# jabberjabberjabber/video-3d-pipeline

Measured on AMD Instinct MI355X. Metric: 1080p_sbs_to_4k_depth_frames_per_s, higher is better.
Workload: dtype int16 (SGM) + f64 (guided filter sums; f32 depth in/out)

## Files before the change

### video-3d-pipeline_amd/csrc/v3d_guided.hip

```cpp
#include "v3d_common.h"
#include <type_traits>

__device__ __forceinline__ double gf_rcp(double x)
{
    double r = __builtin_amdgcn_rcp(x);
    r = fma(r, fma(-x, r, 1.0), r);
    r = fma(r, fma(-x, r, 1.0), r);
    return r;
}

template <typename TD> __device__ __forceinline__ float gf_ld(const TD* p, size_t i);
template <> __device__ __forceinline__ float gf_ld<float>(const float* p, size_t i) { const float v = p[i]; return fabsf(v) <= 3.402823466e38f ? v : 0.f; }
template <> __device__ __forceinline__ float gf_ld<int16_t>(const int16_t* p, size_t i) { const int d = p[i]; return d > 0 ? (float)d * 0.0625f : 0.f; }
template <> __device__ __forceinline__ float gf_ld<uint16_t>(const uint16_t* p, size_t i) { return (float)p[i]; }

typedef unsigned short v3d_u16x2v __attribute__((ext_vector_type(2)));
typedef unsigned short v3d_u16x4 __attribute__((ext_vector_type(4)));
__device__ __forceinline__ void gf_st(float* p, float q) { *p = q; }
__device__ __forceinline__ void gf_st(uint16_t* p, float q) { *p = v3d_rint_u16(q); }

#define GF_TX 64
#define GF_RUN 8
#define GF_RMAX 16

template <typename TD>
__device__ __forceinline__ double gf_bilinear(const TD* __restrict__ src, int Ws, int Hs, double sx, double sy, int x, int y)
{
    const double fx = (x + 0.5) * sx - 0.5, fy = (y + 0.5) * sy - 0.5;
    const double x0f = floor(fx), y0f = floor(fy);
    const double wx = fx - x0f, wy = fy - y0f;
    const int x0 = (int)x0f, y0 = (int)y0f;
    const int xa = min(max(x0, 0), Ws - 1), xb = min(max(x0 + 1, 0), Ws - 1);
    const int ya = min(max(y0, 0), Hs - 1), yb = min(max(y0 + 1, 0), Hs - 1);
    const double top = (double)gf_ld(src, (size_t)ya * Ws + xa) * (1.0 - wx) + (double)gf_ld(src, (size_t)ya * Ws + xb) * wx;
    const double bot = (double)gf_ld(src, (size_t)yb * Ws + xa) * (1.0 - wx) + (double)gf_ld(src, (size_t)yb * Ws + xb) * wx;
    return top * (1.0 - wy) + bot * wy;
}

template <int SWEEP, int GF_RUNY, typename TD, typename TO>
__global__ __launch_bounds__(256) void k_gf(const TD* __restrict__ depth_lo, int Wlo, int Hlo,
                                            const uint8_t* __restrict__ guide, int W, int H, int r, double eps,
                                            double* __restrict__ A, double* __restrict__ B, TO* __restrict__ out)
{
    constexpr int NS = SWEEP == 1 ? 4 : 2;
    constexpr int GF_TY = 4 * GF_RUNY;
    extern __shared__ __attribute__((aligned(16))) double smem[];
    const int rows = GF_TY + 2 * r;
    const int pitch = (GF_TX + 2 * r) | 1;
    const int hp = GF_TX + 1;
    double* t0 = smem;
    double* t1 = t0 + rows * pitch;
    double* hs = t1 + rows * pitch;

    const int tid = threadIdx.x;
    const int ox = blockIdx.x * GF_TX, oy = blockIdx.y * GF_TY;
    const double sx = (double)Wlo / (double)W, sy = (double)Hlo / (double)H;

    const int tw = GF_TX + 2 * r;
    for (int i = tid; i < rows * tw; i += 256) {
        const int ty = i / tw, tx = i - ty * tw;
        const int gx = ox - r + tx, gy = oy - r + ty;
        double v0 = 0.0, v1 = 0.0;
        if (gx >= 0 && gx < W && gy >= 0 && gy < H) {
            if (SWEEP == 1) {
                v0 = (double)guide[(size_t)gy * W + gx] / 255.0;
                v1 = gf_bilinear(depth_lo, Wlo, Hlo, sx, sy, gx, gy);
            } else {
                v0 = A[(size_t)gy * W + gx];
                v1 = B[(size_t)gy * W + gx];
            }
        }
        t0[ty * pitch + tx] = v0;
        t1[ty * pitch + tx] = v1;
    }
    __syncthreads();

    const int nruns = GF_TX / GF_RUN;
    for (int task = tid; task < rows * nruns; task += 256) {
        const int row = task % rows, run = task / rows;
        const double* r0 = t0 + row * pitch + run * GF_RUN;
        const double* r1 = t1 + row * pitch + run * GF_RUN;
        double s0 = 0.0, s1 = 0.0, s2 = 0.0, s3 = 0.0;
        for (int k = 0; k <= 2 * r; k++) {
            const double u = r0[k], v = r1[k];
            s0 += u; s1 += v;
            if (SWEEP == 1) { s2 += u * u; s3 += u * v; }
        }
        double* h = hs + row * hp + run * GF_RUN;
        const int hplane = rows * hp;
        for (int j = 0; j < GF_RUN; j++) {
            h[j] = s0; h[hplane + j] = s1;
            if (SWEEP == 1) { h[2 * hplane + j] = s2; h[3 * hplane + j] = s3; }
            if (j + 1 < GF_RUN) {
                const double un = r0[j + 2 * r + 1], vn = r1[j + 2 * r + 1];
                const double uo = r0[j], vo = r1[j];
                s0 += un - uo; s1 += vn - vo;
                if (SWEEP == 1) { s2 += un * un - uo * uo; s3 += un * vn - uo * vo; }
            }
        }
    }
    __syncthreads();

    {
        const int x = tid % GF_TX, runy = tid / GF_TX;
        const int hplane = rows * hp;
        const double* h = hs + (runy * GF_RUNY) * hp + x;
        double s[NS];
#pragma unroll
        for (int q = 0; q < NS; q++) s[q] = 0.0;
        for (int k = 0; k <= 2 * r; k++)
#pragma unroll
            for (int q = 0; q < NS; q++) s[q] += h[q * hplane + k * hp];
        const int gx = ox + x;
        const int cx = min(gx + r, W - 1) - max(gx - r, 0) + 1;
        for (int j = 0; j < GF_RUNY; j++) {
            const int gy = oy + runy * GF_RUNY + j;
            if (gx < W && gy < H) {
                const int cy = min(gy + r, H - 1) - max(gy - r, 0) + 1;
                const double cnt = (double)(cx * cy);
                if (SWEEP == 1) {
                    const double mI = s[0] / cnt, mp = s[1] / cnt, mII = s[2] / cnt, mIp = s[3] / cnt;
                    const double var = mII - mI * mI, cov = mIp - mI * mp;
                    const double a = cov / (var + eps);
                    A[(size_t)gy * W + gx] = a;
                    B[(size_t)gy * W + gx] = mp - a * mI;
                } else {
                    const double I = (double)guide[(size_t)gy * W + gx] / 255.0;
                    const float q = (float)((s[0] / cnt) * I + (s[1] / cnt));
                    if constexpr (std::is_same<TO, float>::value) out[(size_t)gy * W + gx] = q;
                    else out[(size_t)gy * W + gx] = v3d_rint_u16(q);
                }
            }
            if (j + 1 < GF_RUNY) {
                const int kn = j + 2 * r + 1;
#pragma unroll
                for (int q = 0; q < NS; q++) s[q] += h[q * hplane + kn * hp] - h[q * hplane + j * hp];
            }
        }
    }
}

#ifndef GF_CH
#define GF_CH 3
#endif
typedef double v3d_f64x2 __attribute__((ext_vector_type(2)));
typedef float v3d_f32x2 __attribute__((ext_vector_type(2)));
typedef float v3d_f32x4 __attribute__((ext_vector_type(4)));

template <int SWEEP, int RR, typename TD, typename TO>
__global__ __launch_bounds__(256) void k_gfm(const TD* __restrict__ depth_lo, int Wlo, int Hlo,
                                             const uint8_t* __restrict__ guide, int W, int H, double eps, int band_h,
                                             double* __restrict__ A, double* __restrict__ B, TO* __restrict__ out,
                                             size_t depth_stride, size_t guide_stride)
{
    static_assert(RR % 2 == 0, "pairs must not straddle the strip's halo boundary");
    constexpr int R = 2 * RR + 1, NOUT = 256 - 2 * RR;
    __shared__ __attribute__((aligned(16))) double sVd[2][2][2][256];
    __shared__ __attribute__((aligned(16))) int2 sVi[2][2][256];
    {
        const size_t f = blockIdx.z, n4 = (size_t)W * H;
        depth_lo += f * depth_stride; guide += f * guide_stride; A += f * 2 * n4; B += f * 2 * n4; out += f * n4;
    }
    const int tid = threadIdx.x;
    const int gx = blockIdx.x * NOUT - RR + tid;
    const int ya = blockIdx.y * band_h, yb = min(ya + band_h, H);
    const bool col_ok = gx >= 0 && gx < W;
    const double sx = (double)Wlo / (double)W, sy = (double)Hlo / (double)H;
    const int nsteps = (yb - ya) + 2 * RR;

    const int hrow = tid >> 7, hq = tid & 127;
    const int hgx = blockIdx.x * NOUT - RR + 2 * hq;
    const bool pair_in = 2 * hq >= RR && 2 * hq < 256 - RR;
    const bool px0 = pair_in && hgx < W, px1 = pair_in && hgx + 1 < W;
    const bool vec_ok = px1 && (W & 1) == 0;

    int bxa = 0, bxb = 0; double bwx = 0.0;
    if (SWEEP == 1) {
        const double fx = (gx + 0.5) * sx - 0.5, x0f = floor(fx);
        bwx = fx - x0f;
        bxa = min(max((int)x0f, 0), Wlo - 1); bxb = min(max((int)x0f + 1, 0), Wlo - 1);
    }
    double r0[R], r1[R], v0 = 0.0, v1 = 0.0;
    int rg[R], vg = 0, vgg = 0;
#pragma unroll
    for (int j = 0; j < R; j++) { r0[j] = 0.0; r1[j] = 0.0; rg[j] = 0; }

    struct RowIn { int g; float a0, a1, b0, b1; double n0, n1; bool in; };
    const int gxc = min(max(gx, 0), W - 1);
    auto fetch_row = [&](int t) -> RowIn {
        RowIn q; q.g = 0; q.a0 = q.a1 = q.b0 = q.b1 = 0.f; q.n0 = q.n1 = 0.0;
        const int e = ya - RR + t;
        q.in = col_ok && e >= 0 && e < H && t < nsteps;
        const size_t o = (size_t)min(max(e, 0), H - 1) * W + gxc;
        if (SWEEP == 1) {
            q.g = guide[o];
            const double fy = (e + 0.5) * sy - 0.5, y0f = floor(fy);
            const TD* ra = depth_lo + (size_t)min(max((int)y0f, 0), Hlo - 1) * Wlo;
            const TD* rb = depth_lo + (size_t)min(max((int)y0f + 1, 0), Hlo - 1) * Wlo;
            q.a0 = gf_ld(ra, bxa); q.a1 = gf_ld(ra, bxb); q.b0 = gf_ld(rb, bxa); q.b1 = gf_ld(rb, bxb);
        } else {
            q.n0 = __builtin_nontemporal_load(A + o); q.n1 = __builtin_nontemporal_load(B + o);
        }
        return q;
    };
    RowIn nx[2] = { fetch_row(0), fetch_row(1) };

    int buf = 0;
    for (int t0 = 0; t0 < nsteps; t0 += 2 * R) {
#pragma unroll
        for (int s = 0; s < R; s++) {
            const int tA = t0 + 2 * s;
            if (tA < nsteps) {
                const int y0 = ya - 2 * RR + tA;
                const bool emit = y0 >= ya;
                const RowIn cur[2] = { nx[0], nx[1] };
                nx[0] = fetch_row(tA + 2); nx[1] = fetch_row(tA + 3);
#pragma unroll
                for (int rr = 0; rr < 2; rr++) {
                    const int j = (2 * s + rr) % R;
                    if (SWEEP == 1) {
                        int gn = 0; double pn = 0.0;
                        if (cur[rr].in) {
                            gn = cur[rr].g;
                            const int e = ya - RR + tA + rr;
                            const double fy = (e + 0.5) * sy - 0.5, wy = fy - floor(fy);
                            const double a0 = (double)cur[rr].a0, b0 = (double)cur[rr].b0;
                            const double top = fma(bwx, (double)cur[rr].a1 - a0, a0);
                            const double bot = fma(bwx, (double)cur[rr].b1 - b0, b0);
                            pn = fma(wy, bot - top, top);
                        }
                        const int go = rg[j]; const double po = r1[j];
                        rg[j] = gn; r1[j] = pn;
                        vg += gn - go; vgg += gn * gn - go * go;
                        v0 += pn - po; v1 = fma((double)gn, pn, fma(-(double)go, po, v1));
                    } else {
                        const double n0 = cur[rr].in ? cur[rr].n0 : 0.0, n1 = cur[rr].in ? cur[rr].n1 : 0.0;
                        const double o0 = r0[j], o1 = r1[j];
                        r0[j] = n0; r1[j] = n1;
                        v0 += n0 - o0; v1 += n1 - o1;
                    }
                    if (emit) {
                        sVd[buf][rr][0][tid] = v0; sVd[buf][rr][1][tid] = v1;
                        if (SWEEP == 1) sVi[buf][rr][tid] = make_int2(vg, vgg);
                    }
                }
                if (emit) {
                    __syncthreads();
                    const int y = y0 + hrow;
                    if (px0 && y < yb) {
                        double fq[2], lq[2], cq[2];
#pragma unroll
                        for (int q = 0; q < 2; q++) {
                            const v3d_f64x2* d = reinterpret_cast<const v3d_f64x2*>(&sVd[buf][hrow][q][0]) + (hq - RR / 2);
                            double f = 0.0, l = 0.0, c = 0.0;
#pragma unroll
                            for (int ch = 0; ch <= RR; ch += GF_CH) {
                                v3d_f64x2 w[GF_CH];
#pragma unroll
                                for (int i = 0; i < GF_CH; i++) if (ch + i <= RR) w[i] = d[ch + i];
#pragma unroll
                                for (int i = 0; i < GF_CH; i++) if (ch + i <= RR) {
                                    if (ch + i == 0) { f = w[i].x; c = w[i].y; }
                                    else if (ch + i == RR) { c += w[i].x; l = w[i].y; }
                                    else { c += w[i].x; c += w[i].y; }
                                }
                                asm volatile("" : "+v"(c) :: "memory");
                            }
                            fq[q] = f; lq[q] = l; cq[q] = c;
                        }
                        int g0 = 0, gg0 = 0, gl = 0, ggl = 0, cg = 0, cgg = 0;
                        if (SWEEP == 1) {
                            const int4* gi = reinterpret_cast<const int4*>(&sVi[buf][hrow][0]) + (hq - RR / 2);
#pragma unroll
                            for (int ch = 0; ch <= RR; ch += 3) {
                                int4 u[3];
#pragma unroll
                                for (int i = 0; i < 3; i++) if (ch + i <= RR) u[i] = gi[ch + i];
#pragma unroll
                                for (int i = 0; i < 3; i++) if (ch + i <= RR) {
                                    if (ch + i == 0) { g0 = u[i].x; gg0 = u[i].y; cg = u[i].z; cgg = u[i].w; }
                                    else if (ch + i == RR) { cg += u[i].x; cgg += u[i].y; gl = u[i].z; ggl = u[i].w; }
                                    else { cg += u[i].x + u[i].z; cgg += u[i].y + u[i].w; }
                                }
                                asm volatile("" : "+v"(cg), "+v"(cgg) :: "memory");
                            }
                        }
                        const double s0a = cq[0] + fq[0], s0b = cq[0] + lq[0], s1a = cq[1] + fq[1], s1b = cq[1] + lq[1];
                        const int cy = min(y + RR, H - 1) - max(y - RR, 0) + 1;
                        const int cx0 = min(hgx + RR, W - 1) - max(hgx - RR, 0) + 1, cx1 = min(hgx + 1 + RR, W - 1) - max(hgx + 1 - RR, 0) + 1;
                        const double inva = gf_rcp((double)(cx0 * cy)), invb = cx1 == cx0 ? inva : gf_rcp((double)(cx1 * cy));
                        const size_t o = (size_t)y * W + hgx;
                        if (SWEEP == 1) {
                            const int sga = cg + g0, sgb = cg + gl, sgga = cgg + gg0, sggb = cgg + ggl;
                            double ab[2][2];
#pragma unroll
                            for (int n = 0; n < 2; n++) {
                                const double inv = n ? invb : inva;
                                const double mI = (double)(n ? sgb : sga) * (inv * (1.0 / 255.0)), mp = (n ? s0b : s0a) * inv;
                                const double mII = (double)(n ? sggb : sgga) * (inv * (1.0 / 65025.0)), mIp = (n ? s1b : s1a) * (inv * (1.0 / 255.0));
                                const double var = fma(-mI, mI, mII), cov = fma(-mI, mp, mIp);
                                const double a = cov * gf_rcp(var + eps);
                                ab[n][0] = a; ab[n][1] = fma(-a, mI, mp);
                            }
                            if (vec_ok) {
                                v3d_f64x2 va = { ab[0][0], ab[1][0] }, vb = { ab[0][1], ab[1][1] };
                                __builtin_nontemporal_store(va, reinterpret_cast<v3d_f64x2*>(A + o));
                                __builtin_nontemporal_store(vb, reinterpret_cast<v3d_f64x2*>(B + o));
                            } else {
                                A[o] = ab[0][0]; B[o] = ab[0][1];
                                if (px1) { A[o + 1] = ab[1][0]; B[o + 1] = ab[1][1]; }
                            }
                        } else {
                            const double Ia = (double)guide[o] * (1.0 / 255.0);
                            const double Ib = px1 ? (double)guide[o + 1] * (1.0 / 255.0) : 0.0;
                            const float qa = (float)((s0a * inva) * Ia + (s1a * inva)), qb = (float)((s0b * invb) * Ib + (s1b * invb));
                            if (vec_ok && (std::is_same<TO, float>::value || (reinterpret_cast<uintptr_t>(out + o) & 3) == 0)) {
                                if constexpr (std::is_same<TO, float>::value) {
                                    v3d_f32x2 vq = { qa, qb };
                                    __builtin_nontemporal_store(vq, reinterpret_cast<v3d_f32x2*>(out + o));
                                } else {
                                    v3d_u16x2v vq = { v3d_rint_u16(qa), v3d_rint_u16(qb) };
                                    __builtin_nontemporal_store(vq, reinterpret_cast<v3d_u16x2v*>(out + o));
                                }
                            } else {
                                gf_st(out + o, qa);
                                if (px1) gf_st(out + o + 1, qb);
                            }
                        }
                    }
                    buf ^= 1;
                }
            }
        }
    }
}

__device__ __forceinline__ int gf_swz2(int m) { return m ^ ((m >> 3) & 1) ^ ((m >> 4) & 1); }
__device__ __forceinline__ int gf_swz4(int m) { return m ^ ((m >> 4) & 3); }
__device__ __forceinline__ int gf_c8(int c) { return 2 * gf_swz2(c >> 1) + (c & 1); }

template <int RR>
__device__ __forceinline__ void gf_run4(const double* row, int c0, double s[4])
{
    const v3d_f64x2* d = reinterpret_cast<const v3d_f64x2*>(row);
    const int m0 = (c0 - RR) >> 1;
    double c = 0.0, l0 = 0.0, l1 = 0.0, l2 = 0.0, r1 = 0.0, r2 = 0.0, r3 = 0.0;
#pragma unroll
    for (int k0 = 0; k0 < RR + 2; k0 += GF_CH) {
        v3d_f64x2 w[GF_CH];
#pragma unroll
        for (int i = 0; i < GF_CH; i++) if (k0 + i < RR + 2) w[i] = d[gf_swz2(m0 + k0 + i)];
#pragma unroll
        for (int i = 0; i < GF_CH; i++) {
            const int k = k0 + i;
            if (k == 0) { l0 = w[i].x; l1 = w[i].y; c = w[i].x; c += w[i].y; }
            else if (k == 1) { l2 = w[i].x; c += w[i].x; c += w[i].y; }
            else if (k < RR) { c += w[i].x; c += w[i].y; }
            else if (k == RR) { c += w[i].x; r1 = w[i].y; }
            else if (k == RR + 1) { r2 = w[i].x; r3 = w[i].y; }
        }
        asm volatile("" : "+v"(c) :: "memory");
    }
    s[0] = c; s[1] = (s[0] + r1) - l0; s[2] = (s[1] + r2) - l1; s[3] = (s[2] + r3) - l2;
}

template <int RR>
__device__ __forceinline__ void gf_run4(const int2* row, int c0, int2 s[4])
{
    const int4* d = reinterpret_cast<const int4*>(row);
    const int m0 = (c0 - RR) >> 1;
    int2 c = make_int2(0, 0), l0 = c, l1 = c, l2 = c, r1 = c, r2 = c, r3 = c;
#pragma unroll
    for (int k0 = 0; k0 < RR + 2; k0 += 3) {
        int4 w[3];
#pragma unroll
        for (int i = 0; i < 3; i++) if (k0 + i < RR + 2) w[i] = d[gf_swz2(m0 + k0 + i)];
#pragma unroll
        for (int i = 0; i < 3; i++) {
            const int k = k0 + i;
            const int2 a = make_int2(w[i].x, w[i].y), b = make_int2(w[i].z, w[i].w);
            if (k == 0) { l0 = a; l1 = b; c = make_int2(a.x + b.x, a.y + b.y); }
            else if (k == 1) { l2 = a; c.x += a.x + b.x; c.y += a.y + b.y; }
            else if (k < RR) { c.x += a.x + b.x; c.y += a.y + b.y; }
            else if (k == RR) { c.x += a.x; c.y += a.y; r1 = b; }
            else if (k == RR + 1) { r2 = a; r3 = b; }
        }
        asm volatile("" : "+v"(c.x), "+v"(c.y) :: "memory");
    }
    s[0] = c;
    s[1] = make_int2(s[0].x + r1.x - l0.x, s[0].y + r1.y - l0.y);
    s[2] = make_int2(s[1].x + r2.x - l1.x, s[1].y + r2.y - l1.y);
    s[3] = make_int2(s[2].x + r3.x - l2.x, s[2].y + r3.y - l2.y);
}

template <int RR>
__device__ __forceinline__ void gf_run4(const int4* row, int c0, int4 s[4])
{
    int4 c = make_int4(0, 0, 0, 0), l0 = c, l1 = c, l2 = c, r1 = c, r2 = c, r3 = c;
#pragma unroll
    for (int k0 = 0; k0 < 2 * RR + 4; k0 += 3) {
        int4 u[3];
#pragma unroll
        for (int i = 0; i < 3; i++) if (k0 + i < 2 * RR + 4) u[i] = row[gf_swz4(c0 - RR + k0 + i)];
#pragma unroll
        for (int i = 0; i < 3; i++) {
            const int k = k0 + i;
            if (k < 2 * RR + 1) { c.x += u[i].x; c.y += u[i].y; c.z += u[i].z; c.w += u[i].w; }
            if (k == 0) l0 = u[i];
            else if (k == 1) l1 = u[i];
            else if (k == 2) l2 = u[i];
            else if (k == 2 * RR + 1) r1 = u[i];
            else if (k == 2 * RR + 2) r2 = u[i];
            else if (k == 2 * RR + 3) r3 = u[i];
        }
        asm volatile("" : "+v"(c.x), "+v"(c.y), "+v"(c.z), "+v"(c.w) :: "memory");
    }
    s[0] = c;
    s[1] = make_int4(s[0].x - l0.x + r1.x, s[0].y - l0.y + r1.y, s[0].z - l0.z + r1.z, s[0].w - l0.w + r1.w);
    s[2] = make_int4(s[1].x - l1.x + r2.x, s[1].y - l1.y + r2.y, s[1].z - l1.z + r2.z, s[1].w - l1.w + r2.w);
    s[3] = make_int4(s[2].x - l2.x + r3.x, s[2].y - l2.y + r3.y, s[2].z - l2.z + r3.z, s[2].w - l2.w + r3.w);
}

template <int RR>
__device__ __forceinline__ void gf_solve4(const int sg[4], const int sgg[4], const double sp[4], const double sgp[4], int hgx, int y,
                                          int W, int H, double eps, double a[4], double b[4])
{
    const int cy = min(y + RR, H - 1) - max(y - RR, 0) + 1;
    int cx[4];
#pragma unroll
    for (int n = 0; n < 4; n++) cx[n] = min(hgx + n + RR, W - 1) - max(hgx + n - RR, 0) + 1;
    const double inv0 = gf_rcp((double)(cx[0] * cy));
#pragma unroll
    for (int n = 0; n < 4; n++) {
        const double inv = (n == 0 || cx[n] == cx[0]) ? inv0 : gf_rcp((double)(cx[n] * cy));
        const double mI = (double)sg[n] * (inv * (1.0 / 255.0)), mp = sp[n] * inv;
        const double mII = (double)sgg[n] * (inv * (1.0 / 65025.0)), mIp = sgp[n] * (inv * (1.0 / 255.0));
        const double var = fma(-mI, mI, mII), cov = fma(-mI, mp, mIp);
        const double aa = cov * gf_rcp(var + eps);
        a[n] = aa; b[n] = fma(-aa, mI, mp);
    }
}

template <int RR, int COLS, typename TD, bool I1, typename TO>
__global__ __launch_bounds__(2 * COLS, I1 ? 4 : 2) void k_gff(const TD* __restrict__ depth_lo, int Wlo, int Hlo,
                                                const uint8_t* __restrict__ guide, int W, int H, double eps, int band_h,
                                                TO* __restrict__ out, size_t depth_stride, size_t guide_stride)
{
    static_assert(RR % 4 == 0, "runs of four must not straddle the strip's halo boundaries");
    static_assert(!I1 || std::is_same<TD, int16_t>::value, "the integer stage 1 takes the int16 disparity");
    static_assert(COLS == 256 || (COLS == 512 && I1), "strip width (512 columns: I1 only, the f64 route's rows exceed the LDS)");
    constexpr int R = 2 * RR + 1, NOUT = COLS - 4 * RR, HR = COLS / 4;
    constexpr int S1D = 2 * 4 * 2 * COLS * 8, S1 = I1 ? 2 * 4 * COLS * 16 : S1D + 2 * 4 * COLS * 8;
    __shared__ __attribute__((aligned(16))) unsigned char sS1[S1];
    double (*sV1)[4][2][COLS] = reinterpret_cast<double (*)[4][2][COLS]>(sS1);
    int2 (*sVi)[4][COLS] = reinterpret_cast<int2 (*)[4][COLS]>(sS1 + (I1 ? 0 : S1D));
    int4 (*sVq)[4][COLS] = reinterpret_cast<int4 (*)[4][COLS]>(sS1);
    (void)sV1; (void)sVi; (void)sVq;
    __shared__ __attribute__((aligned(16))) double sAB[3][4][2][COLS];
    {
        const size_t f = blockIdx.z, n4 = (size_t)W * H;
        depth_lo += f * depth_stride; guide += f * guide_stride; out += f * n4;
    }
    const int role = __builtin_amdgcn_readfirstlane((int)(threadIdx.x / COLS));
    const int t = threadIdx.x % COLS;
    const int gx0 = blockIdx.x * NOUT - 2 * RR;
    const int gx = gx0 + t;
    const int ya = blockIdx.y * band_h, yb = min(ya + band_h, H);
    const int nrows = (yb - ya) + 4 * RR;
    const int NS = (nrows + 3) >> 2;
    const int NP = NS + 3;

    if (role == 0) {
        const bool col_ok = gx >= 0 && gx < W;
        const int gxc = min(max(gx, 0), W - 1);
        uint32_t ring[R];
        double r1[I1 ? 1 : R];
        uint32_t rgw[I1 ? 1 : (R + 3) / 4];
        int vg = 0, vgg = 0, vP = 0, vgP = 0;
        double v0 = 0.0, v1 = 0.0;
#pragma unroll
        for (int j = 0; j < R; j++) ring[j] = 0u;
#pragma unroll
        for (int j = 0; j < (I1 ? 1 : R); j++) r1[j] = 0.0;
#pragma unroll
        for (int j = 0; j < (I1 ? 1 : (R + 3) / 4); j++) rgw[j] = 0u;
        (void)ring; (void)r1; (void)rgw;
        int bxa, bxb, wxa = 0, wxb = 0; double bwx = 0.0;
        const double sx = (double)Wlo / (double)W, sy = (double)Hlo / (double)H;
        if constexpr (I1) {
            const int kx = gx >> 1;
            bxa = min(max((gx & 1) ? kx : kx - 1, 0), Wlo - 1); bxb = min(max((gx & 1) ? kx + 1 : kx, 0), Wlo - 1);
            wxa = (gx & 1) ? 3 : 1; wxb = 4 - wxa;
        } else {
            const double fx = (gx + 0.5) * sx - 0.5, x0f = floor(fx);
            bwx = fx - x0f;
            bxa = min(max((int)x0f, 0), Wlo - 1); bxb = min(max((int)x0f + 1, 0), Wlo - 1);
        }
        (void)wxa; (void)wxb; (void)bwx;
        struct RowIn { int g; typename std::conditional<I1, int, float>::type a0, a1, b0, b1; bool in; };
        auto fetch_row = [&](int tt) -> RowIn {
            RowIn q;
            const int e = ya - 2 * RR + tt;
            q.in = col_ok && e >= 0 && e < H && tt < nrows;
            const int ec = min(max(e, 0), H - 1);
            q.g = guide[(size_t)ec * W + gxc];
            if constexpr (I1) {
                const int ky = ec >> 1;
                const TD* ra = depth_lo + (size_t)min(max((ec & 1) ? ky : ky - 1, 0), Hlo - 1) * Wlo;
                const TD* rb = depth_lo + (size_t)min(max((ec & 1) ? ky + 1 : ky, 0), Hlo - 1) * Wlo;
                q.a0 = max((int)ra[bxa], 0); q.a1 = max((int)ra[bxb], 0); q.b0 = max((int)rb[bxa], 0); q.b1 = max((int)rb[bxb], 0);
            } else {
                const double fy = (e + 0.5) * sy - 0.5, y0f = floor(fy);
                const TD* ra = depth_lo + (size_t)min(max((int)y0f, 0), Hlo - 1) * Wlo;
                const TD* rb = depth_lo + (size_t)min(max((int)y0f + 1, 0), Hlo - 1) * Wlo;
                q.a0 = gf_ld(ra, bxa); q.a1 = gf_ld(ra, bxb); q.b0 = gf_ld(rb, bxa); q.b1 = gf_ld(rb, bxb);
            }
            return q;
        };
        RowIn nx[4] = { fetch_row(0), fetch_row(1), fetch_row(2), fetch_row(3) };
        for (int p0 = 0; p0 < NP; p0 += R) {
#pragma clang loop unroll(full)
            for (int sp = 0; sp < R; sp++) {
                const int p = p0 + sp;
                if (p < NP) {
                    int tl = t;
                    asm volatile("" : "+v"(tl));
                    const int hrow = tl / HR, c0 = 4 * (tl % HR), hgx = gx0 + c0;
                    const int j = p - 1;
                    if (j >= RR / 2 && j < NS) {
                        const int y = ya - 3 * RR + 4 * j + hrow;
                        double a[4] = { 0.0, 0.0, 0.0, 0.0 }, b[4] = { 0.0, 0.0, 0.0, 0.0 };
                        if (c0 >= RR && c0 < COLS - RR && y >= 0 && y < H && hgx >= 0 && hgx < W) {
                            int sg[4], sgg[4]; double sp_[4], sgp[4];
                            if constexpr (I1) {
                                int4 s[4];
                                gf_run4<RR>(&sVq[j & 1][hrow][0], c0, s);
#pragma unroll
                                for (int n = 0; n < 4; n++) {
                                    sg[n] = s[n].x; sgg[n] = s[n].y;
                                    sp_[n] = (double)s[n].z * (1.0 / 256.0); sgp[n] = (double)s[n].w * (1.0 / 256.0);
                                }
                            } else {
                                int2 si[4];
                                gf_run4<RR>(&sVi[j & 1][hrow][0], c0, si);
                                gf_run4<RR>(&sV1[j & 1][hrow][0][0], c0, sp_);
                                gf_run4<RR>(&sV1[j & 1][hrow][1][0], c0, sgp);
#pragma unroll
                                for (int n = 0; n < 4; n++) { sg[n] = si[n].x; sgg[n] = si[n].y; }
                            }
                            gf_solve4<RR>(sg, sgg, sp_, sgp, hgx, y, W, H, eps, a, b);
#pragma unroll
                            for (int n = 0; n < 4; n++) if (hgx + n >= W) { a[n] = 0.0; b[n] = 0.0; }
                        }
                        double* ab = &sAB[j % 3][hrow][0][0];
                        const int e0 = 2 * gf_swz2(c0 >> 1), e1 = 2 * gf_swz2((c0 >> 1) + 1);
                        *reinterpret_cast<v3d_f64x2*>(ab + e0) = v3d_f64x2{ a[0], a[1] };
                        *reinterpret_cast<v3d_f64x2*>(ab + e1) = v3d_f64x2{ a[2], a[3] };
                        *reinterpret_cast<v3d_f64x2*>(ab + COLS + e0) = v3d_f64x2{ b[0], b[1] };
                        *reinterpret_cast<v3d_f64x2*>(ab + COLS + e1) = v3d_f64x2{ b[2], b[3] };
                    }
                    if (p < NS) {
                        const int tA = 4 * p;
                        const RowIn cur[4] = { nx[0], nx[1], nx[2], nx[3] };
#pragma unroll
                        for (int k = 0; k < 4; k++) nx[k] = fetch_row(tA + 4 + k);
                        const bool emit = p >= RR / 2;
#pragma unroll
                        for (int rr = 0; rr < 4; rr++) {
                            const int slot = (4 * sp + rr) % R;
                            const int e = ya - 2 * RR + tA + rr;
                            if constexpr (I1) {
                                int gn = 0, Pn = 0;
                                if (cur[rr].in) {
                                    gn = cur[rr].g;
                                    const int wya = (e & 1) ? 3 : 1;
                                    Pn = wya * (wxa * cur[rr].a0 + wxb * cur[rr].a1) + (4 - wya) * (wxa * cur[rr].b0 + wxb * cur[rr].b1);
                                }
                                const int go = (int)(ring[slot] & 0xFFu), Po = (int)(ring[slot] >> 8);
                                ring[slot] = ((uint32_t)Pn << 8) | (uint32_t)gn;
                                vg += gn - go; vgg += gn * gn - go * go;
                                vP += Pn - Po; vgP += gn * Pn - go * Po;
                                if (emit) sVq[p & 1][rr][gf_swz4(t)] = make_int4(vg, vgg, vP, vgP);
                            } else {
                                int gn = 0; double pn = 0.0;
                                if (cur[rr].in) {
                                    gn = cur[rr].g;
                                    const double fy = (e + 0.5) * sy - 0.5, wy = fy - floor(fy);
                                    const double a0 = (double)cur[rr].a0, b0 = (double)cur[rr].b0;
                                    const double top = fma(bwx, (double)cur[rr].a1 - a0, a0);
                                    const double bot = fma(bwx, (double)cur[rr].b1 - b0, b0);
                                    pn = fma(wy, bot - top, top);
                                }
                                const int go = (int)((rgw[slot >> 2] >> (8 * (slot & 3))) & 0xFFu); const double po = r1[slot];
                                rgw[slot >> 2] = (rgw[slot >> 2] & ~(0xFFu << (8 * (slot & 3)))) | ((uint32_t)gn << (8 * (slot & 3)));
                                r1[slot] = pn;
                                vg += gn - go; vgg += gn * gn - go * go;
                                v0 += pn - po; v1 = fma((double)gn, pn, fma(-(double)go, po, v1));
                                if (emit) {
                                    const int ct = gf_c8(t);
                                    sV1[p & 1][rr][0][ct] = v0; sV1[p & 1][rr][1][ct] = v1;
                                    sVi[p & 1][rr][ct] = make_int2(vg, vgg);
                                }
                            }
                        }
                    }
                    __syncthreads();
                }
            }
        }
    } else {
        double r0[R], r1[R], va = 0.0, vb = 0.0;
#pragma unroll
        for (int j = 0; j < R; j++) { r0[j] = 0.0; r1[j] = 0.0; }
        for (int p0 = 0; p0 < NP; p0 += R) {
#pragma clang loop unroll(full)
            for (int sp = 0; sp < R; sp++) {
                const int p = p0 + sp;
                if (p < NP) {
                    int tl = t;
                    asm volatile("" : "+v"(tl));
                    const int hrow = tl / HR, c0 = 4 * (tl % HR), hgx = gx0 + c0;
                    {
                        const int j = p - 3;
                        const int y = ya - 4 * RR + 4 * j + hrow;
                        if (j >= RR && j < NS && c0 >= 2 * RR && c0 < COLS - 2 * RR && hgx < W && y < yb) {
                            double sa[4], sb[4];
                            gf_run4<RR>(&sAB[j % 3][hrow][0][0], c0, sa);
                            gf_run4<RR>(&sAB[j % 3][hrow][1][0], c0, sb);
                            const int cy = min(y + RR, H - 1) - max(y - RR, 0) + 1;
                            int cx[4];
#pragma unroll
                            for (int n = 0; n < 4; n++) cx[n] = min(hgx + n + RR, W - 1) - max(hgx + n - RR, 0) + 1;
                            const double inv0 = gf_rcp((double)(cx[0] * cy));
                            const size_t o = (size_t)y * W + hgx;
                            const bool all_in = hgx + 3 < W;
                            const bool vec_ok = all_in && (W & 3) == 0 && ((reinterpret_cast<uintptr_t>(out + o) | reinterpret_cast<uintptr_t>(guide + o)) & 3) == 0
                                                && (reinterpret_cast<uintptr_t>(out + o) & (4 * sizeof(TO) - 1)) == 0;
                            int g[4];
                            if (vec_ok) {
                                const uint32_t g4 = *reinterpret_cast<const uint32_t*>(guide + o);
#pragma unroll
                                for (int n = 0; n < 4; n++) g[n] = (g4 >> (8 * n)) & 0xFF;
                            } else {
#pragma unroll
                                for (int n = 0; n < 4; n++) g[n] = hgx + n < W ? guide[o + n] : 0;
                            }
                            float q[4];
#pragma unroll
                            for (int n = 0; n < 4; n++) {
                                const double inv = (n == 0 || cx[n] == cx[0]) ? inv0 : gf_rcp((double)(cx[n] * cy));
                                const double I = (double)g[n] * (1.0 / 255.0);
                                q[n] = (float)((sa[n] * inv) * I + (sb[n] * inv));
                            }
                            if (vec_ok) {
                                if constexpr (std::is_same<TO, float>::value) {
                                    const v3d_f32x4 vq = { q[0], q[1], q[2], q[3] };
                                    __builtin_nontemporal_store(vq, reinterpret_cast<v3d_f32x4*>(out + o));
                                } else {
                                    const v3d_u16x4 vq = { v3d_rint_u16(q[0]), v3d_rint_u16(q[1]), v3d_rint_u16(q[2]), v3d_rint_u16(q[3]) };
                                    __builtin_nontemporal_store(vq, reinterpret_cast<v3d_u16x4*>(out + o));
                                }
                            } else {
#pragma unroll
                                for (int n = 0; n < 4; n++) if (hgx + n < W) gf_st(out + o + n, q[n]);
                            }
                        }
                    }
                    {
                        const int j = p - 2;
                        if (j >= RR / 2 && j < NS) {
                            const bool emit = j >= RR;
                            double* col = &sAB[j % 3][0][0][gf_c8(tl)];
#pragma unroll
                            for (int rr = 0; rr < 4; rr++) {
                                const int slot = (4 * sp + rr) % R;
                                const double n0 = col[rr * 2 * COLS], n1 = col[rr * 2 * COLS + COLS];
                                const double o0 = r0[slot], o1 = r1[slot];
                                r0[slot] = n0; r1[slot] = n1;
                                va += n0 - o0; vb += n1 - o1;
                                if (emit) { col[rr * 2 * COLS] = va; col[rr * 2 * COLS + COLS] = vb; }
                            }
                        }
                    }
                    __syncthreads();
                }
            }
        }
    }
}

template <int RR, typename TD, typename TO>
static void launch_gff(const TD* depth_lo, int Wlo, int Hlo, const uint8_t* guide, int W, int H, double eps,
                       TO* out, int n, size_t depth_stride, size_t guide_stride, hipStream_t st)
{
    bool i1 = false;
    if constexpr (std::is_same<TD, int16_t>::value) i1 = g_v3d_opt.gf_int1 && W == 2 * Wlo && H == 2 * Hlo;
    const int cols = g_v3d_opt.gf_cols == 512 && i1 ? 512 : 256;
    int band = g_v3d_opt.gf_band;
    if (band <= 0) {
        int dev = 0, ncu = 256;
        (void)hipGetDevice(&dev);
        (void)hipDeviceGetAttribute(&ncu, hipDeviceAttributeMultiprocessorCount, dev);
        const long slots = (long)ncu * (cols == 256 && i1 ? 2 : 1), strips = v3d_cdiv(W, cols - 4 * RR);
        long best = -1;
        for (int nb = 1; nb <= 64 && nb <= H; nb++) {
            const int b = (v3d_cdiv(H, nb) + 1) & ~1;
            const long wgs = strips * v3d_cdiv(H, b) * n, rounds = (wgs + slots - 1) / slots, cost = rounds * (b + 4 * RR);
            if (best < 0 || cost < best) { best = cost; band = b; }
        }
    }
    const dim3 grid(v3d_cdiv(W, cols - 4 * RR), v3d_cdiv(H, band), n);
    if constexpr (std::is_same<TD, int16_t>::value) {
        if (i1 && cols == 512) {
            hipLaunchKernelGGL((k_gff<RR, 512, TD, true, TO>), grid, dim3(1024), 0, st, depth_lo, Wlo, Hlo, guide, W, H, eps, band, out, depth_stride, guide_stride);
            return;
        }
        if (i1) {
            hipLaunchKernelGGL((k_gff<RR, 256, TD, true, TO>), grid, dim3(512), 0, st, depth_lo, Wlo, Hlo, guide, W, H, eps, band, out, depth_stride, guide_stride);
            return;
        }
    }
    hipLaunchKernelGGL((k_gff<RR, 256, TD, false, TO>), grid, dim3(512), 0, st, depth_lo, Wlo, Hlo, guide, W, H, eps, band, out, depth_stride, guide_stride);
}

template <int RR, typename TD, typename TO>
static void launch_gfm(const TD* depth_lo, int Wlo, int Hlo, const uint8_t* guide, int W, int H, double eps,
                       double* A, double* B, TO* out, int n, size_t depth_stride, size_t guide_stride, hipStream_t st)
{
    const int band1 = g_v3d_opt.gf_band1, band2 = g_v3d_opt.gf_band2;
    const dim3 grid1(v3d_cdiv(W, 256 - 2 * RR), v3d_cdiv(H, band1), n), grid2(v3d_cdiv(W, 256 - 2 * RR), v3d_cdiv(H, band2), n);
    hipLaunchKernelGGL((k_gfm<1, RR, TD, TO>), grid1, dim3(256), 0, st, depth_lo, Wlo, Hlo, guide, W, H, eps, band1, A, B, out, depth_stride, guide_stride);
    hipLaunchKernelGGL((k_gfm<2, RR, TD, TO>), grid2, dim3(256), 0, st, depth_lo, Wlo, Hlo, guide, W, H, eps, band2, A, B, out, depth_stride, guide_stride);
}

extern "C" size_t v3d_guided_upscale_ws_bytes(int W, int H)
{
    if (W < 1 || H < 1) return 0;
    return (size_t)W * H * sizeof(double) * 2;
}

static size_t gf_smem(int r, int ns, int ty)
{
    const int rows = ty + 2 * r;
    const int pitch = (GF_TX + 2 * r) | 1;
    return sizeof(double) * ((size_t)2 * rows * pitch + (size_t)ns * rows * (GF_TX + 1));
}

template <typename TD, typename TO>
static int guided_upscale_batch(const TD* depth_lo, int Wlo, int Hlo, size_t depth_stride, const uint8_t* guide,
                                int W, int H, size_t guide_stride, int n, int r, float eps, TO* out, void* ws, void* stream)
{
    if (n < 1) { v3d_set_error("bad batch"); return V3D_ERR_ARG; }
    if (!depth_lo || !guide || !out || !ws) { v3d_set_error("null pointer"); return V3D_ERR_ARG; }
    if (Wlo < 1 || Hlo < 1 || W < 1 || H < 1) { v3d_set_error("bad geometry"); return V3D_ERR_ARG; }
    if (r < 1 || r > GF_RMAX) { v3d_set_error("radius %d outside [1, %d]", r, GF_RMAX); return V3D_ERR_UNSUPPORTED; }
    if (!(eps >= 0.f)) { v3d_set_error("eps must be >= 0"); return V3D_ERR_ARG; }
    if (((uintptr_t)ws & 15) != 0) { v3d_set_error("workspace must be 16-byte aligned"); return V3D_ERR_ARG; }
    hipStream_t st = (hipStream_t)stream;
    double* A = reinterpret_cast<double*>(ws);
    double* B = A + (size_t)W * H;
    if (!g_v3d_opt.gf_tiled && g_v3d_opt.gf_fused && (r == 4 || r == 8)) {
        if (r == 4) launch_gff<4>(depth_lo, Wlo, Hlo, guide, W, H, (double)eps, out, n, depth_stride, guide_stride, st);
        else launch_gff<8>(depth_lo, Wlo, Hlo, guide, W, H, (double)eps, out, n, depth_stride, guide_stride, st);
        V3D_LAUNCH_CHECK();
        return V3D_OK;
    }
    if (!g_v3d_opt.gf_tiled && (r == 4 || r == 8)) {
        if (r == 4) launch_gfm<4>(depth_lo, Wlo, Hlo, guide, W, H, (double)eps, A, B, out, n, depth_stride, guide_stride, st);
        else launch_gfm<8>(depth_lo, Wlo, Hlo, guide, W, H, (double)eps, A, B, out, n, depth_stride, guide_stride, st);
        V3D_LAUNCH_CHECK();
        return V3D_OK;
    }
    for (int f = 0; f < n; f++) {
    const TD* depth_lo_f = depth_lo + (size_t)f * depth_stride; const uint8_t* guide_f = guide + (size_t)f * guide_stride;
    double* A = reinterpret_cast<double*>(ws) + (size_t)f * 2 * W * H; double* B = A + (size_t)W * H; TO* out_f = out + (size_t)f * W * H;
    const int ty = r <= 8 ? 16 : 8;
    const dim3 grid(v3d_cdiv(W, GF_TX), v3d_cdiv(H, ty));
    const size_t sm1 = gf_smem(r, 4, ty), sm2 = gf_smem(r, 2, ty);
    if (ty == 16) {
        V3D_HIP_CHECK(hipFuncSetAttribute((const void*)k_gf<1, 4, TD, TO>, hipFuncAttributeMaxDynamicSharedMemorySize, (int)sm1));
        V3D_HIP_CHECK(hipFuncSetAttribute((const void*)k_gf<2, 4, TD, TO>, hipFuncAttributeMaxDynamicSharedMemorySize, (int)sm2));
        hipLaunchKernelGGL((k_gf<1, 4, TD, TO>), grid, dim3(256), sm1, st, depth_lo_f, Wlo, Hlo, guide_f, W, H, r, (double)eps, A, B, out_f);
        hipLaunchKernelGGL((k_gf<2, 4, TD, TO>), grid, dim3(256), sm2, st, depth_lo_f, Wlo, Hlo, guide_f, W, H, r, (double)eps, A, B, out_f);
    } else {
        V3D_HIP_CHECK(hipFuncSetAttribute((const void*)k_gf<1, 2, TD, TO>, hipFuncAttributeMaxDynamicSharedMemorySize, (int)sm1));
        V3D_HIP_CHECK(hipFuncSetAttribute((const void*)k_gf<2, 2, TD, TO>, hipFuncAttributeMaxDynamicSharedMemorySize, (int)sm2));
        hipLaunchKernelGGL((k_gf<1, 2, TD, TO>), grid, dim3(256), sm1, st, depth_lo_f, Wlo, Hlo, guide_f, W, H, r, (double)eps, A, B, out_f);
        hipLaunchKernelGGL((k_gf<2, 2, TD, TO>), grid, dim3(256), sm2, st, depth_lo_f, Wlo, Hlo, guide_f, W, H, r, (double)eps, A, B, out_f);
    }
    }
    V3D_LAUNCH_CHECK();
    return V3D_OK;
}

extern "C" int v3d_guided_upscale_batch(const float* depth_lo, int Wlo, int Hlo, size_t depth_stride, const uint8_t* guide,
                                        int W, int H, size_t guide_stride, int n, int r, float eps, float* out, void* ws, void* stream)
{
    return guided_upscale_batch<float, float>(depth_lo, Wlo, Hlo, depth_stride, guide, W, H, guide_stride, n, r, eps, out, ws, stream);
}

extern "C" int v3d_guided_upscale(const float* depth_lo, int Wlo, int Hlo, const uint8_t* guide, int W, int H,
                                  int r, float eps, float* out, void* ws, void* stream)
{
    return guided_upscale_batch<float, float>(depth_lo, Wlo, Hlo, 0, guide, W, H, 0, 1, r, eps, out, ws, stream);
}

extern "C" int v3d_guided_upscale_disp16_batch(const int16_t* disp16, int Wlo, int Hlo, size_t disp_stride, const uint8_t* guide,
                                               int W, int H, size_t guide_stride, int n, int r, float eps, float* out, void* ws, void* stream)
{
    return guided_upscale_batch<int16_t, float>(disp16, Wlo, Hlo, disp_stride, guide, W, H, guide_stride, n, r, eps, out, ws, stream);
}

extern "C" int v3d_guided_upscale_u16_batch(const uint16_t* depth_lo, int Wlo, int Hlo, size_t depth_stride, const uint8_t* guide,
                                            int W, int H, size_t guide_stride, int n, int r, float eps, uint16_t* out, void* ws, void* stream)
{
    return guided_upscale_batch<uint16_t, uint16_t>(depth_lo, Wlo, Hlo, depth_stride, guide, W, H, guide_stride, n, r, eps, out, ws, stream);
}
```

Measured before the change: 2563.

## Add interior fast path and scalar row addressing to the guided filter kernel

Adds a wave-uniform interior fast path that uses a precomputed full-window reciprocal instead of per-pixel clipped box counts and f64 reciprocals, in both the coefficient solve and the output stage. The row fetch is restructured to load four rows per step, with scalar (SGPR) row base pointers and 32-bit byte offsets. In the integer route the 2x upsampled bilinear weights are computed once per step from shared horizontal sums using 24-bit multiply-add inline asm, and hrow is made wave-uniform via readfirstlane. This trims VALU address and f64 work in a compute-heavy kernel, at the cost of more inline asm, register pressure and code size.

```diff
diff --git a/video-3d-pipeline_amd/csrc/v3d_guided.hip b/video-3d-pipeline_amd/csrc/v3d_guided.hip
--- a/video-3d-pipeline_amd/csrc/v3d_guided.hip
+++ b/video-3d-pipeline_amd/csrc/v3d_guided.hip
@@ -9,10 +9,22 @@
     return r;
 }
 
-template <typename TD> __device__ __forceinline__ float gf_ld(const TD* p, size_t i);
-template <> __device__ __forceinline__ float gf_ld<float>(const float* p, size_t i) { const float v = p[i]; return fabsf(v) <= 3.402823466e38f ? v : 0.f; }
-template <> __device__ __forceinline__ float gf_ld<int16_t>(const int16_t* p, size_t i) { const int d = p[i]; return d > 0 ? (float)d * 0.0625f : 0.f; }
-template <> __device__ __forceinline__ float gf_ld<uint16_t>(const uint16_t* p, size_t i) { return (float)p[i]; }
+__device__ __forceinline__ float gf_val(float v) { return fabsf(v) <= 3.402823466e38f ? v : 0.f; }
+__device__ __forceinline__ float gf_val(int16_t v) { const int d = v; return d > 0 ? (float)d * 0.0625f : 0.f; }
+__device__ __forceinline__ float gf_val(uint16_t v) { return (float)v; }
+template <typename TD> __device__ __forceinline__ float gf_ld(const TD* p, size_t i) { return gf_val(p[i]); }
+
+#define GF_GLOBAL __attribute__((address_space(1)))
+template <typename T> __device__ __forceinline__ const GF_GLOBAL T* gf_srow(const T* p)
+{
+    const GF_GLOBAL T* g = (const GF_GLOBAL T*)p;
+    asm("" : "+s"(g));
+    return g;
+}
+template <typename T> __device__ __forceinline__ T gf_at(const GF_GLOBAL T* row, uint32_t byte_off)
+{
+    return *reinterpret_cast<const GF_GLOBAL T*>(reinterpret_cast<const GF_GLOBAL char*>(row) + byte_off);
+}
 
 typedef unsigned short v3d_u16x2v __attribute__((ext_vector_type(2)));
 typedef unsigned short v3d_u16x4 __attribute__((ext_vector_type(4)));
@@ -421,6 +433,31 @@
     s[3] = make_int4(s[2].x - l2.x + r3.x, s[2].y - l2.y + r3.y, s[2].z - l2.z + r3.z, s[2].w - l2.w + r3.w);
 }
 
+__device__ __forceinline__ double gf_uniform(double x)
+{
+    const uint64_t v = (uint64_t)__double_as_longlong(x);
+    const uint32_t lo = __builtin_amdgcn_readfirstlane((uint32_t)v), hi = __builtin_amdgcn_readfirstlane((uint32_t)(v >> 32));
+    return __longlong_as_double((long long)(((uint64_t)hi << 32) | lo));
+}
+
+template <int RR>
+__device__ __forceinline__ double gf_inv_full()
+{
+    int n = (2 * RR + 1) * (2 * RR + 1);
+    asm volatile("" : "+v"(n));
+    return gf_uniform(gf_rcp((double)n));
+}
+
+__device__ __forceinline__ void gf_ab(int sg, int sgg, double sp, double sgp, double inv, double inv255, double inv65025,
+                                      double eps, double& a, double& b)
+{
+    const double mI = (double)sg * inv255, mp = sp * inv;
+    const double mII = (double)sgg * inv65025, mIp = sgp * inv255;
+    const double var = fma(-mI, mI, mII), cov = fma(-mI, mp, mIp);
+    const double aa = cov * gf_rcp(var + eps);
+    a = aa; b = fma(-aa, mI, mp);
+}
+
 template <int RR>
 __device__ __forceinline__ void gf_solve4(const int sg[4], const int sgg[4], const double sp[4], const double sgp[4], int hgx, int y,
                                           int W, int H, double eps, double a[4], double b[4])
@@ -429,16 +466,25 @@
     int cx[4];
 #pragma unroll
     for (int n = 0; n < 4; n++) cx[n] = min(hgx + n + RR, W - 1) - max(hgx + n - RR, 0) + 1;
-    const double inv0 = gf_rcp((double)(cx[0] * cy));
+    const double inv0 = gf_rcp((double)__mul24(cx[0], cy));
 #pragma unroll
     for (int n = 0; n < 4; n++) {
-        const double inv = (n == 0 || cx[n] == cx[0]) ? inv0 : gf_rcp((double)(cx[n] * cy));
-        const double mI = (double)sg[n] * (inv * (1.0 / 255.0)), mp = sp[n] * inv;
-        const double mII = (double)sgg[n] * (inv * (1.0 / 65025.0)), mIp = sgp[n] * (inv * (1.0 / 255.0));
-        const double var = fma(-mI, mI, mII), cov = fma(-mI, mp, mIp);
-        const double aa = cov * gf_rcp(var + eps);
-        a[n] = aa; b[n] = fma(-aa, mI, mp);
-    }
+        const double inv = (n == 0 || cx[n] == cx[0]) ? inv0 : gf_rcp((double)__mul24(cx[n], cy));
+        gf_ab(sg[n], sgg[n], sp[n], sgp[n], inv, inv * (1.0 / 255.0), inv * (1.0 / 65025.0), eps, a[n], b[n]);
+    }
+}
+
+__device__ __forceinline__ int gf_mad24(int a, int b, int c)
+{
+    int d;
+    asm("v_mad_i32_i24 %0, %1, %2, %3" : "=v"(d) : "v"(a), "v"(b), "v"(c));
+    return d;
+}
+__device__ __forceinline__ int gf_mad24x3(int a, int c)
+{
+    int d;
+    asm("v_mad_i32_i24 %0, %1, 3, %2" : "=v"(d) : "v"(a), "v"(c));
+    return d;
 }
 
 template <int RR, int COLS, typename TD, bool I1, typename TO>
@@ -450,6 +496,7 @@
     static_assert(!I1 || std::is_same<TD, int16_t>::value, "the integer stage 1 takes the int16 disparity");
     static_assert(COLS == 256 || (COLS == 512 && I1), "strip width (512 columns: I1 only, the f64 route's rows exceed the LDS)");
     constexpr int R = 2 * RR + 1, NOUT = COLS - 4 * RR, HR = COLS / 4;
+    static_assert(HR % 64 == 0, "the lanes of a wave work on one row in the horizontal phases");
     constexpr int S1D = 2 * 4 * 2 * COLS * 8, S1 = I1 ? 2 * 4 * COLS * 16 : S1D + 2 * 4 * COLS * 8;
     __shared__ __attribute__((aligned(16))) unsigned char sS1[S1];
     double (*sV1)[4][2][COLS] = reinterpret_cast<double (*)[4][2][COLS]>(sS1);
@@ -462,13 +509,15 @@
         depth_lo += f * depth_stride; guide += f * guide_stride; out += f * n4;
     }
     const int role = __builtin_amdgcn_readfirstlane((int)(threadIdx.x / COLS));
-    const int t = threadIdx.x % COLS;
+    int t = threadIdx.x % COLS;
+    asm volatile("" : "+v"(t));
     const int gx0 = blockIdx.x * NOUT - 2 * RR;
     const int gx = gx0 + t;
     const int ya = blockIdx.y * band_h, yb = min(ya + band_h, H);
     const int nrows = (yb - ya) + 4 * RR;
     const int NS = (nrows + 3) >> 2;
     const int NP = NS + 3;
+    const double invF = gf_inv_full<RR>();
 
     if (role == 0) {
         const bool col_ok = gx >= 0 && gx < W;
@@ -485,39 +534,48 @@
 #pragma unroll
         for (int j = 0; j < (I1 ? 1 : (R + 3) / 4); j++) rgw[j] = 0u;
         (void)ring; (void)r1; (void)rgw;
-        int bxa, bxb, wxa = 0, wxb = 0; double bwx = 0.0;
+        uint32_t oxg = (uint32_t)gxc, oxa, oxb; double bwx = 0.0;
         const double sx = (double)Wlo / (double)W, sy = (double)Hlo / (double)H;
         if constexpr (I1) {
             const int kx = gx >> 1;
-            bxa = min(max((gx & 1) ? kx : kx - 1, 0), Wlo - 1); bxb = min(max((gx & 1) ? kx + 1 : kx, 0), Wlo - 1);
-            wxa = (gx & 1) ? 3 : 1; wxb = 4 - wxa;
+            oxa = (uint32_t)min(max((gx & 1) ? kx + 1 : kx - 1, 0), Wlo - 1) * (uint32_t)sizeof(TD);
+            oxb = (uint32_t)min(max(kx, 0), Wlo - 1) * (uint32_t)sizeof(TD);
         } else {
             const double fx = (gx + 0.5) * sx - 0.5, x0f = floor(fx);
             bwx = fx - x0f;
-            bxa = min(max((int)x0f, 0), Wlo - 1); bxb = min(max((int)x0f + 1, 0), Wlo - 1);
-        }
-        (void)wxa; (void)wxb; (void)bwx;
-        struct RowIn { int g; typename std::conditional<I1, int, float>::type a0, a1, b0, b1; bool in; };
-        auto fetch_row = [&](int tt) -> RowIn {
-            RowIn q;
-            const int e = ya - 2 * RR + tt;
-            q.in = col_ok && e >= 0 && e < H && tt < nrows;
-            const int ec = min(max(e, 0), H - 1);
-            q.g = guide[(size_t)ec * W + gxc];
+            oxa = (uint32_t)min(max((int)x0f, 0), Wlo - 1) * (uint32_t)sizeof(TD);
+            oxb = (uint32_t)min(max((int)x0f + 1, 0), Wlo - 1) * (uint32_t)sizeof(TD);
+        }
+        (void)bwx;
+        struct StepIn { int g[4]; typename std::conditional<I1, int, float>::type d[I1 ? 4 : 8][2]; };
+        auto fetch_step = [&](int tt) -> StepIn {
+            StepIn q;
+            const int e0 = ya - 2 * RR + tt;
+            asm volatile("" : "+v"(oxg), "+v"(oxa), "+v"(oxb));
+#pragma unroll
+            for (int k = 0; k < 4; k++) q.g[k] = gf_at(gf_srow(guide + (size_t)min(max(e0 + k, 0), H - 1) * W), oxg);
             if constexpr (I1) {
-                const int ky = ec >> 1;
-                const TD* ra = depth_lo + (size_t)min(max((ec & 1) ? ky : ky - 1, 0), Hlo - 1) * Wlo;
-                const TD* rb = depth_lo + (size_t)min(max((ec & 1) ? ky + 1 : ky, 0), Hlo - 1) * Wlo;
-                q.a0 = max((int)ra[bxa], 0); q.a1 = max((int)ra[bxb], 0); q.b0 = max((int)rb[bxa], 0); q.b1 = max((int)rb[bxb], 0);
+                const int kb = (e0 >> 1) - 1;
+#pragma unroll
+                for (int i = 0; i < 4; i++) {
+                    const auto row = gf_srow(depth_lo + (size_t)min(max(kb + i, 0), Hlo - 1) * Wlo);
+                    q.d[i][0] = max((int)gf_at(row, oxa), 0); q.d[i][1] = max((int)gf_at(row, oxb), 0);
+                }
             } else {
-                const double fy = (e + 0.5) * sy - 0.5, y0f = floor(fy);
-                const TD* ra = depth_lo + (size_t)min(max((int)y0f, 0), Hlo - 1) * Wlo;
-                const TD* rb = depth_lo + (size_t)min(max((int)y0f + 1, 0), Hlo - 1) * Wlo;
-                q.a0 = gf_ld(ra, bxa); q.a1 = gf_ld(ra, bxb); q.b0 = gf_ld(rb, bxa); q.b1 = gf_ld(rb, bxb);
+#pragma unroll
+                for (int k = 0; k < 4; k++) {
+                    const int ec = min(max(e0 + k, 0), H - 1);
+                    const double fy = (ec + 0.5) * sy - 0.5, y0f = floor(fy);
+                    const auto ra = gf_srow(depth_lo + (size_t)min(max((int)y0f, 0), Hlo - 1) * Wlo);
+                    const auto rb = gf_srow(depth_lo + (size_t)min(max((int)y0f + 1, 0), Hlo - 1) * Wlo);
+                    q.d[2 * k][0] = gf_val(gf_at(ra, oxa)); q.d[2 * k][1] = gf_val(gf_at(ra, oxb));
+                    q.d[2 * k + 1][0] = gf_val(gf_at(rb, oxa)); q.d[2 * k + 1][1] = gf_val(gf_at(rb, oxb));
+                }
             }
             return q;
         };
-        RowIn nx[4] = { fetch_row(0), fetch_row(1), fetch_row(2), fetch_row(3) };
+        const double invF255 = gf_uniform(invF * (1.0 / 255.0)), invF65025 = gf_uniform(invF * (1.0 / 65025.0));
+        StepIn nx = fetch_step(0);
         for (int p0 = 0; p0 < NP; p0 += R) {
 #pragma clang loop unroll(full)
             for (int sp = 0; sp < R; sp++) {
@@ -525,7 +583,8 @@
                 if (p < NP) {
                     int tl = t;
                     asm volatile("" : "+v"(tl));
-                    const int hrow = tl / HR, c0 = 4 * (tl % HR), hgx = gx0 + c0;
+                    const int hrow = __builtin_amdgcn_readfirstlane(tl / HR);
+                    const int c0 = 4 * (tl % HR), hgx = gx0 + c0;
                     const int j = p - 1;
                     if (j >= RR / 2 && j < NS) {
                         const int y = ya - 3 * RR + 4 * j + hrow;
@@ -548,9 +607,15 @@
 #pragma unroll
                                 for (int n = 0; n < 4; n++) { sg[n] = si[n].x; sgg[n] = si[n].y; }
                             }
-                            gf_solve4<RR>(sg, sgg, sp_, sgp, hgx, y, W, H, eps, a, b);
-#pragma unroll
-                            for (int n = 0; n < 4; n++) if (hgx + n >= W) { a[n] = 0.0; b[n] = 0.0; }
+                            const bool clipped = y < RR || y + RR >= H || hgx < RR || hgx + 3 + RR >= W;
+                            if (!__any(clipped)) {
+#pragma unroll
+                                for (int n = 0; n < 4; n++) gf_ab(sg[n], sgg[n], sp_[n], sgp[n], invF, invF255, invF65025, eps, a[n], b[n]);
+                            } else {
+                                gf_solve4<RR>(sg, sgg, sp_, sgp, hgx, y, W, H, eps, a, b);
+#pragma unroll
+                                for (int n = 0; n < 4; n++) if (hgx + n >= W) { a[n] = 0.0; b[n] = 0.0; }
+                            }
                         }
                         double* ab = &sAB[j % 3][hrow][0][0];
                         const int e0 = 2 * gf_swz2(c0 >> 1), e1 = 2 * gf_swz2((c0 >> 1) + 1);
@@ -561,40 +626,50 @@
                     }
                     if (p < NS) {
                         const int tA = 4 * p;
-                        const RowIn cur[4] = { nx[0], nx[1], nx[2], nx[3] };
-#pragma unroll
-                        for (int k = 0; k < 4; k++) nx[k] = fetch_row(tA + 4 + k);
+                        const StepIn cur = nx;
+                        nx = fetch_step(tA + 4);
                         const bool emit = p >= RR / 2;
+                        const int e0 = ya - 2 * RR + tA;
+                        int Pq[4];
+                        if constexpr (I1) {
+                            static_assert(sizeof(TD) == 2 && 16 * 32767 < (1 << 23), "P = 256 p must be a signed 24-bit operand");
+                            int h[4];
+#pragma unroll
+                            for (int i = 0; i < 4; i++) h[i] = gf_mad24x3(cur.d[i][1], cur.d[i][0]);
+                            if (e0 & 1) {
+                                Pq[0] = gf_mad24x3(h[1], h[2]); Pq[1] = gf_mad24x3(h[2], h[1]); Pq[2] = gf_mad24x3(h[2], h[3]); Pq[3] = gf_mad24x3(h[3], h[2]);
+                            } else {
+                                Pq[0] = gf_mad24x3(h[1], h[0]); Pq[1] = gf_mad24x3(h[1], h[2]); Pq[2] = gf_mad24x3(h[2], h[1]); Pq[3] = gf_mad24x3(h[2], h[3]);
+                            }
+                        }
+                        (void)Pq;
 #pragma unroll
                         for (int rr = 0; rr < 4; rr++) {
                             const int slot = (4 * sp + rr) % R;
-                            const int e = ya - 2 * RR + tA + rr;
+                            const int e = e0 + rr;
+                            const bool in = col_ok && e >= 0 && e < H && tA + rr < nrows;
                             if constexpr (I1) {
                                 int gn = 0, Pn = 0;
-                                if (cur[rr].in) {
-                                    gn = cur[rr].g;
-                                    const int wya = (e & 1) ? 3 : 1;
-                                    Pn = wya * (wxa * cur[rr].a0 + wxb * cur[rr].a1) + (4 - wya) * (wxa * cur[rr].b0 + wxb * cur[rr].b1);
-                                }
-                                const int go = (int)(ring[slot] & 0xFFu), Po = (int)(ring[slot] >> 8);
+                                if (in) { gn = cur.g[rr]; Pn = Pq[rr]; }
+                                const int go = (int)(ring[slot] & 0xFFu), Po = (int)(ring[slot] >> 8), ngo = -go;
                                 ring[slot] = ((uint32_t)Pn << 8) | (uint32_t)gn;
-                                vg += gn - go; vgg += gn * gn - go * go;
-                                vP += Pn - Po; vgP += gn * Pn - go * Po;
+                                vg += gn - go; vgg = gf_mad24(ngo, go, gf_mad24(gn, gn, vgg));
+                                vP += Pn - Po; vgP = gf_mad24(ngo, Po, gf_mad24(gn, Pn, vgP));
                                 if (emit) sVq[p & 1][rr][gf_swz4(t)] = make_int4(vg, vgg, vP, vgP);
                             } else {
                                 int gn = 0; double pn = 0.0;
-                                if (cur[rr].in) {
-                                    gn = cur[rr].g;
+                                if (in) {
+                                    gn = cur.g[rr];
                                     const double fy = (e + 0.5) * sy - 0.5, wy = fy - floor(fy);
-                                    const double a0 = (double)cur[rr].a0, b0 = (double)cur[rr].b0;
-                                    const double top = fma(bwx, (double)cur[rr].a1 - a0, a0);
-                                    const double bot = fma(bwx, (double)cur[rr].b1 - b0, b0);
+                                    const double a0 = (double)cur.d[2 * rr][0], b0 = (double)cur.d[2 * rr + 1][0];
+                                    const double top = fma(bwx, (double)cur.d[2 * rr][1] - a0, a0);
+                                    const double bot = fma(bwx, (double)cur.d[2 * rr + 1][1] - b0, b0);
                                     pn = fma(wy, bot - top, top);
                                 }
                                 const int go = (int)((rgw[slot >> 2] >> (8 * (slot & 3))) & 0xFFu); const double po = r1[slot];
                                 rgw[slot >> 2] = (rgw[slot >> 2] & ~(0xFFu << (8 * (slot & 3)))) | ((uint32_t)gn << (8 * (slot & 3)));
                                 r1[slot] = pn;
-                                vg += gn - go; vgg += gn * gn - go * go;
+                                vg += gn - go; vgg = gf_mad24(-go, go, gf_mad24(gn, gn, vgg));
                                 v0 += pn - po; v1 = fma((double)gn, pn, fma(-(double)go, po, v1));
                                 if (emit) {
                                     const int ct = gf_c8(t);
@@ -619,7 +694,8 @@
                 if (p < NP) {
                     int tl = t;
                     asm volatile("" : "+v"(tl));
-                    const int hrow = tl / HR, c0 = 4 * (tl % HR), hgx = gx0 + c0;
+                    const int hrow = __builtin_amdgcn_readfirstlane(tl / HR);
+                    const int c0 = 4 * (tl % HR), hgx = gx0 + c0;
                     {
                         const int j = p - 3;
                         const int y = ya - 4 * RR + 4 * j + hrow;
@@ -627,11 +703,6 @@
                             double sa[4], sb[4];
                             gf_run4<RR>(&sAB[j % 3][hrow][0][0], c0, sa);
                             gf_run4<RR>(&sAB[j % 3][hrow][1][0], c0, sb);
-                            const int cy = min(y + RR, H - 1) - max(y - RR, 0) + 1;
-                            int cx[4];
-#pragma unroll
-                            for (int n = 0; n < 4; n++) cx[n] = min(hgx + n + RR, W - 1) - max(hgx + n - RR, 0) + 1;
-                            const double inv0 = gf_rcp((double)(cx[0] * cy));
                             const size_t o = (size_t)y * W + hgx;
                             const bool all_in = hgx + 3 < W;
                             const bool vec_ok = all_in && (W & 3) == 0 && ((reinterpret_cast<uintptr_t>(out + o) | reinterpret_cast<uintptr_t>(guide + o)) & 3) == 0
@@ -646,11 +717,24 @@
                                 for (int n = 0; n < 4; n++) g[n] = hgx + n < W ? guide[o + n] : 0;
                             }
                             float q[4];
-#pragma unroll
-                            for (int n = 0; n < 4; n++) {
-                                const double inv = (n == 0 || cx[n] == cx[0]) ? inv0 : gf_rcp((double)(cx[n] * cy));
-                                const double I = (double)g[n] * (1.0 / 255.0);
-                                q[n] = (float)((sa[n] * inv) * I + (sb[n] * inv));
+                            if (!__any(y < RR || y + RR >= H || hgx < RR || hgx + 3 + RR >= W)) {
+#pragma unroll
+                                for (int n = 0; n < 4; n++) {
+                                    const double I = (double)g[n] * (1.0 / 255.0);
+                                    q[n] = (float)((sa[n] * invF) * I + (sb[n] * invF));
+                                }
+                            } else {
+                                const int cy = min(y + RR, H - 1) - max(y - RR, 0) + 1;
+                                int cx[4];
+#pragma unroll
+                                for (int n = 0; n < 4; n++) cx[n] = min(hgx + n + RR, W - 1) - max(hgx + n - RR, 0) + 1;
+                                const double inv0 = gf_rcp((double)__mul24(cx[0], cy));
+#pragma unroll
+                                for (int n = 0; n < 4; n++) {
+                                    const double inv = (n == 0 || cx[n] == cx[0]) ? inv0 : gf_rcp((double)__mul24(cx[n], cy));
+                                    const double I = (double)g[n] * (1.0 / 255.0);
+                                    q[n] = (float)((sa[n] * inv) * I + (sb[n] * inv));
+                                }
                             }
                             if (vec_ok) {
                                 if constexpr (std::is_same<TO, float>::value) {
```

After: 2594 (median of 6 runs). 1.01x the previous value.
